# MrTornado24/IDE-3D

Measured on AMD Instinct MI355X. Metric: 512x512 RGB+seg frames/s @96 depth samples (whole job), higher is better.
Workload: dtype f32 (3x3 convs + MLPs: fp32 operands as 3 bf16 pieces, 6 products, f32 accumulate); 1 GPU; BASELINE config 2: random-init ide3d-ffhq-64-512, G.mapping + G.synthesis (64 render -> 512, 96 samples, RGB + 19-class seg) + uint8 frames, batch 4 seeds per GPU; global_batch=4, parallelism=dp1, conv_arithmetic=bf16x6, conv_arithmetic_is_library_default=True

## Files before the change

### ide-3d_amd/csrc/upfirdn2d.hip

```cpp
#include "common.h"
#include "knobs.h"
#include <type_traits>

namespace ide3d {

template <class T>
__device__ __forceinline__ typename Elem<T>::math_t
apply_epilogue(typename Elem<T>::math_t v, const ide3d_upfirdn2d_epilogue& ep, int n, int c, int oy, int ox, int out_w) {
    using M = typename Elem<T>::math_t;
    if (ep.add) v += Elem<T>::ld((const T*)ep.add + n * ep.add_stride[0] + c * ep.add_stride[1] + oy * ep.add_stride[2] + ox * ep.add_stride[3]);
    if (ep.noise) v += (M)(ep.noise[oy * out_w + ox] * ep.noise_strength);
    if (ep.fused_act) {
        if (ep.bias) v += Elem<T>::ld((const T*)ep.bias + c);
        if (ep.act == 3) v = (v > 0) ? v : v * (M)ep.alpha;
        v *= (M)ep.act_gain;
        if (ep.clamp >= 0.f) v = (v > (M)ep.clamp) ? (M)ep.clamp : ((v < -(M)ep.clamp) ? -(M)ep.clamp : v);
    }
    return v;
}

template <class T, int NO>
__device__ __forceinline__ void epilogue_row(typename Elem<T>::math_t (&row)[NO], const ide3d_upfirdn2d_epilogue& ep,
                                             const T* add_plane, typename Elem<T>::math_t bias, int oy, int ox0, int out_w, bool full) {
    using M = typename Elem<T>::math_t;
    if (ep.add) {
        const T* ap = add_plane + (int64_t)oy * ep.add_stride[2];
        if constexpr (sizeof(T) == 4 && NO == 4) {
            if (full && ep.add_stride[3] == 1 && ((reinterpret_cast<uintptr_t>(ap + ox0) & 15) == 0)) {
                const float4 a = *reinterpret_cast<const float4*>(ap + ox0);
                row[0] += a.x; row[1] += a.y; row[2] += a.z; row[3] += a.w;
                goto add_done;
            }
        }
#pragma unroll
        for (int j = 0; j < NO; ++j) {
            const int ox = ox0 + j;
            if (ox >= 0 && ox < out_w) row[j] += Elem<T>::ld(ap + (int64_t)ox * ep.add_stride[3]);
        }
    }
add_done:
    if (ep.noise) {
        const float* np_ = ep.noise + (int64_t)oy * out_w;
        if (NO == 4 && full && ((reinterpret_cast<uintptr_t>(np_ + ox0) & 15) == 0)) {
            const float4 a = *reinterpret_cast<const float4*>(np_ + ox0);
            row[0] += (M)(a.x * ep.noise_strength); row[1] += (M)(a.y * ep.noise_strength);
            row[2] += (M)(a.z * ep.noise_strength); row[3] += (M)(a.w * ep.noise_strength);
        } else {
#pragma unroll
            for (int j = 0; j < NO; ++j) {
                const int ox = ox0 + j;
                if (ox >= 0 && ox < out_w) row[j] += (M)(np_[ox] * ep.noise_strength);
            }
        }
    }
    if (ep.fused_act) {
#pragma unroll
        for (int j = 0; j < NO; ++j) {
            M v = row[j] + bias;
            if (ep.act == 3) v = (v > 0) ? v : v * (M)ep.alpha;
            v *= (M)ep.act_gain;
            if (ep.clamp >= 0.f) v = (v > (M)ep.clamp) ? (M)ep.clamp : ((v < -(M)ep.clamp) ? -(M)ep.clamp : v);
            row[j] = v;
        }
    }
}


template <class T>
__global__ void __launch_bounds__(256)
upfirdn2d_generic_kernel(ide3d_upfirdn2d_params p, ide3d_upfirdn2d_epilogue ep, int c_fastest) {
    using M = typename Elem<T>::math_t;
    const T* __restrict__ x = (const T*)p.x;
    T* __restrict__ y = (T*)p.y;
    const int64_t total = (int64_t)p.n * p.c * p.out_h * p.out_w;
    const int64_t stride = (int64_t)gridDim.x * blockDim.x;
    int am_n = -1; float am = 0.f;
    __shared__ unsigned s_am[64];
    const bool am_lds = ep.y_amax && p.n <= 64;
    if (ep.y_amax) { if (threadIdx.x < 64) s_am[threadIdx.x] = 0u; __syncthreads(); }
    for (int64_t idx = (int64_t)blockIdx.x * blockDim.x + threadIdx.x; idx < total; idx += stride) {
        int ox, oy, c, n;
        int64_t r = idx;
        if (c_fastest) {
            c = (int)(r % p.c); r /= p.c;
            ox = (int)(r % p.out_w); r /= p.out_w;
            oy = (int)(r % p.out_h); r /= p.out_h;
            n = (int)r;
        } else {
            ox = (int)(r % p.out_w); r /= p.out_w;
            oy = (int)(r % p.out_h); r /= p.out_h;
            c = (int)(r % p.c); r /= p.c;
            n = (int)r;
        }
        const int X0 = ox * p.down_x - p.pad_x0;
        const int Y0 = oy * p.down_y - p.pad_y0;
        int kx0, ky0, ix0, iy0;
        if (p.up_x == 1) { kx0 = 0; ix0 = X0; } else { ix0 = floordiv(X0 + p.up_x - 1, p.up_x); kx0 = ix0 * p.up_x - X0; }
        if (p.up_y == 1) { ky0 = 0; iy0 = Y0; } else { iy0 = floordiv(Y0 + p.up_y - 1, p.up_y); ky0 = iy0 * p.up_y - Y0; }
        int ty_begin = 0, tx_begin = 0;
        if (iy0 < 0) ty_begin = -iy0;
        if (ix0 < 0) tx_begin = -ix0;
        const int ty_end = min((p.f_h - ky0 + p.up_y - 1) / p.up_y, p.in_h - iy0);
        const int tx_end = min((p.f_w - kx0 + p.up_x - 1) / p.up_x, p.in_w - ix0);
        const T* xp = x + n * p.x_stride[0] + c * p.x_stride[1];
        M acc = 0;
        for (int ty = ty_begin; ty < ty_end; ++ty) {
            const int ky = ky0 + ty * p.up_y;
            const int fy = p.flip ? ky : p.f_h - 1 - ky;
            const T* xr = xp + (int64_t)(iy0 + ty) * p.x_stride[2];
            const float* fr = p.f + (int64_t)fy * p.f_stride[0];
            int kx = kx0 + tx_begin * p.up_x;
            for (int tx = tx_begin; tx < tx_end; ++tx, kx += p.up_x) {
                const int fx = p.flip ? kx : p.f_w - 1 - kx;
                acc += Elem<T>::ld(xr + (int64_t)(ix0 + tx) * p.x_stride[3]) * (M)fr[fx * p.f_stride[1]];
            }
        }
        const M out = apply_epilogue<T>(acc * (M)p.gain, ep, n, c, oy, ox, p.out_w);
        Elem<T>::st(y + n * p.y_stride[0] + c * p.y_stride[1] + oy * p.y_stride[2] + ox * p.y_stride[3], out);
        if (ep.y_amax) {
            if (n != am_n) { if (am_n >= 0) { if (am_lds) amax_lds_flush(s_am, am_n, am); else if (am > 0.f) amax_raise(ep.y_amax, am_n, am); } am_n = n; am = 0.f; }
            am = fmaxf(am, fabsf((float)out));
        }
    }
    if (ep.y_amax) {
        if (am_n >= 0) { if (am_lds) amax_lds_flush(s_am, am_n, am); else if (am > 0.f) amax_raise(ep.y_amax, am_n, am); }
        if (am_lds) amax_lds_commit(ep.y_amax, s_am, p.n);
    }
}

__host__ __device__ inline int cell_row_floats(int ntx, int U) { return ((ntx + 1 + 7) / 8) * 8 * U; }

template <class T, int U>
__global__ void __launch_bounds__(256)
upfirdn2d_cell_kernel(ide3d_upfirdn2d_params p, ide3d_upfirdn2d_epilogue ep, int cells_x, int cells_y, int qx_min, int qy_min, int ntx, int nty) {
    using M = typename Elem<T>::math_t;
    extern __shared__ __attribute__((aligned(16))) float s_fpad[];
    const int FPW = cell_row_floats(ntx, U), FPH = (nty + 1) * U;
    for (int e = threadIdx.x; e < FPW * FPH; e += 256) {
        const int ky = e / FPW - (U - 1), kx = e % FPW - (U - 1);
        float v = 0.f;
        if (ky >= 0 && ky < p.f_h && kx >= 0 && kx < p.f_w) {
            const int fy = p.flip ? ky : p.f_h - 1 - ky, fx = p.flip ? kx : p.f_w - 1 - kx;
            v = p.f[(int64_t)fy * p.f_stride[0] + (int64_t)fx * p.f_stride[1]];
        }
        s_fpad[e] = v;
    }
    __syncthreads();
    const T* __restrict__ x = (const T*)p.x;
    T* __restrict__ y = (T*)p.y;
    const int64_t total = (int64_t)p.n * p.c * cells_y * U * cells_x;
    const int64_t stride = (int64_t)gridDim.x * blockDim.x;
    for (int64_t idx = (int64_t)blockIdx.x * blockDim.x + threadIdx.x; idx < total; idx += stride) {
        int64_t r = idx;
        const int cxi = (int)(r % cells_x); r /= cells_x;
        const int jy = (int)(r % U); r /= U;
        const int cyi = (int)(r % cells_y); r /= cells_y;
        const int c = (int)(r % p.c), n = (int)(r / p.c);
        const int qx = qx_min + cxi, qy = qy_min + cyi;
        const int oy = qy * U + jy + p.pad_y0;
        if (oy < 0 || oy >= p.out_h) continue;
        M acc[U];
#pragma unroll
        for (int jx = 0; jx < U; ++jx) acc[jx] = 0;
        const T* xp = x + n * p.x_stride[0] + c * p.x_stride[1];
        for (int dy = 0; dy <= nty; ++dy) {
            const int iy = qy + dy;
            if (iy < 0 || iy >= p.in_h) continue;
            const T* xr = xp + (int64_t)iy * p.x_stride[2];
            const float* frow = s_fpad + (dy * U + U - 1 - jy) * FPW;
            const int s3 = (int)p.x_stride[3];
            for (int dx0 = 0; dx0 <= ntx; dx0 += 8) {
                M xv[8];
#pragma unroll
                for (int e = 0; e < 8; ++e) {
                    const int ix = qx + dx0 + e;
                    const bool ok = (unsigned)ix < (unsigned)p.in_w;
                    const M v = Elem<T>::ld(xr + (ok ? ix : 0) * s3);
                    xv[e] = ok ? v : (M)0;
                }
                const float* fb = frow + dx0 * U;
#pragma unroll
                for (int e = 0; e < 8; ++e) {
#pragma unroll
                    for (int jx = 0; jx < U; ++jx) acc[jx] += xv[e] * (M)fb[e * U + U - 1 - jx];
                }
            }
        }
#pragma unroll
        for (int jx = 0; jx < U; ++jx) {
            const int ox = qx * U + jx + p.pad_x0;
            if (ox < 0 || ox >= p.out_w) continue;
            const M out = apply_epilogue<T>(acc[jx] * (M)p.gain, ep, n, c, oy, ox, p.out_w);
            Elem<T>::st(y + n * p.y_stride[0] + c * p.y_stride[1] + oy * p.y_stride[2] + ox * p.y_stride[3], out);
        }
    }
}


template <int U, int D, int F>
struct Axis {
    static constexpr int NT = (F + U - 1) / U;
    static constexpr int first(int r) { return (U - r) % U; }
    static constexpr int ntaps(int r) { return first(r) < F ? (F - first(r) + U - 1) / U : 0; }
    static constexpr int off(int r) { return r == 0 ? 0 : 1; }
    static constexpr int window(int C) { return U > 1 ? C + NT : (C - 1) * D + F; }
    static constexpr int step = (U > 1) ? 1 : D;
};

template <int UX, int UY, int DX, int DY, int FW, int FH, int CX, int CY>
struct TileGeom {
    using AX = Axis<UX, DX, FW>;
    using AY = Axis<UY, DY, FH>;
    static constexpr int TX = 32, TY = 8;
    static constexpr int TCX = TX * CX, TCY = TY * CY;
    static constexpr int LW = ((AX::window(TCX) + 3) & ~3) + 4;
    static constexpr int LH = AY::window(TCY);
    static constexpr int NLD4 = (LH * (LW / 4) + 255) / 256;
};

__host__ __device__ constexpr bool tile_stage16_instance(int elem_bytes, int nld4) { return elem_bytes == 4 && nld4 <= 16; }
__host__ __device__ inline bool tile_stage16_plane(int64_t pitch, int in_w, int x_row_floats, uintptr_t plane_addr) {
    const int w4 = (in_w + 3) & ~3;
    return (pitch & 3) == 0 && pitch >= w4 && w4 <= (in_w > x_row_floats ? in_w : x_row_floats) && (plane_addr & 15) == 0;
}

template <class T, int UX, int UY, int DX, int DY, int FW, int FH, int CX, int CY>
__global__ void __launch_bounds__(256)
upfirdn2d_tile_kernel(ide3d_upfirdn2d_params p, ide3d_upfirdn2d_epilogue ep, int tiles_x, int tiles_y) {
    using M = typename Elem<T>::math_t;
    using G = TileGeom<UX, UY, DX, DY, FW, FH, CX, CY>;
    using AX = typename G::AX;
    using AY = typename G::AY;
    constexpr int TX = G::TX;
    constexpr int TCX = G::TCX, TCY = G::TCY;
    constexpr int LW = G::LW, LH = G::LH;
    constexpr int WX = AX::window(CX), WY = AY::window(CY);

    __shared__ __attribute__((aligned(16))) M s_in[LH * LW];

    M g[FH][FW];
#pragma unroll
    for (int ky = 0; ky < FH; ++ky)
#pragma unroll
        for (int kx = 0; kx < FW; ++kx) {
            const int fy = p.flip ? ky : FH - 1 - ky;
            const int fx = p.flip ? kx : FW - 1 - kx;
            g[ky][kx] = (M)p.f[fy * p.f_stride[0] + fx * p.f_stride[1]] * (M)p.gain;
        }

    const int nblocks = gridDim.x;
    int bid = xcd_remap(blockIdx.x, nblocks);
    const int tx_i = bid % tiles_x; bid /= tiles_x;
    const int ty_i = bid % tiles_y; bid /= tiles_y;
    const int plane = bid;
    const int n = plane / p.c, c = plane % p.c;

    const int qx_min = (UX > 1) ? floordiv(-p.pad_x0, UX) : 0;
    const int qy_min = (UY > 1) ? floordiv(-p.pad_y0, UY) : 0;
    const int qx0 = qx_min + tx_i * TCX;
    const int qy0 = qy_min + ty_i * TCY;
    const int in_x0 = (UX > 1) ? qx0 : qx0 * DX - p.pad_x0;
    const int in_y0 = (UY > 1) ? qy0 : qy0 * DY - p.pad_y0;

    const T* __restrict__ xp = (const T*)p.x + n * p.x_stride[0] + c * p.x_stride[1];
    int xoff = 0;
    bool staged = false;
    if constexpr (tile_stage16_instance((int)sizeof(T), G::NLD4)) {
        const int64_t pitch = p.x_stride[2];
        const int w4 = (p.in_w + 3) & ~3;
        if (tile_stage16_plane(pitch, p.in_w, p.x_row_floats, reinterpret_cast<uintptr_t>(xp))) {
            const int x_al = in_x0 & ~3;
            xoff = in_x0 - x_al;
            constexpr int NV = LW / 4, NLD4 = (LH * NV + 255) / 256;
            static_assert(LW % 4 == 0 && LW >= AX::window(TCX) + 4, "LDS rows hold the window shifted by up to 3 columns");
            float4 v4[NLD4];
            unsigned long long okb = 0;
#pragma unroll
            for (int k = 0; k < NLD4; ++k) {
                const int idx = (int)threadIdx.x + k * 256;
                const int ly = idx / NV, lv = idx - ly * NV;
                const int gy = in_y0 + ly, gx = x_al + 4 * lv;
                const int cy_ = min(max(gy, 0), p.in_h - 1), cxv = min(max(gx, 0), w4 - 4);
                v4[k] = *reinterpret_cast<const float4*>(reinterpret_cast<const float*>(xp) + (int64_t)cy_ * pitch + cxv);
                const bool rowok = (gy == cy_) && idx < LH * NV;
#pragma unroll
                for (int e = 0; e < 4; ++e) okb |= (rowok && gx + e >= 0 && gx + e < p.in_w) ? (1ull << (4 * k + e)) : 0ull;
            }
#pragma unroll
            for (int k = 0; k < NLD4; ++k) {
                const int idx = (int)threadIdx.x + k * 256;
                if (idx < LH * NV) {
                    float4 w = v4[k];
                    w.x = ((okb >> (4 * k + 0)) & 1ull) ? w.x : 0.f; w.y = ((okb >> (4 * k + 1)) & 1ull) ? w.y : 0.f;
                    w.z = ((okb >> (4 * k + 2)) & 1ull) ? w.z : 0.f; w.w = ((okb >> (4 * k + 3)) & 1ull) ? w.w : 0.f;
                    *reinterpret_cast<float4*>(reinterpret_cast<float*>(s_in) + 4 * idx) = w;
                }
            }
            staged = true;
        }
    }
    if (!staged) {
        constexpr int NLD = (LH * LW + 255) / 256;
        constexpr int DROW = 256 / LW, DCOL = 256 % LW;
        M v[NLD];
        int ly = (int)threadIdx.x / LW, lx = (int)threadIdx.x % LW;
        static_assert(NLD <= 64, "staging loads per thread must fit the validity mask");
        unsigned long long okbits = 0;
#pragma unroll
        for (int k = 0; k < NLD; ++k) {
            const int iy = in_y0 + ly, ix = in_x0 + lx;
            const int cy_ = min(max(iy, 0), p.in_h - 1), cx_ = min(max(ix, 0), p.in_w - 1);
            v[k] = Elem<T>::ld(xp + cy_ * p.x_stride[2] + cx_);
            okbits |= (lx < AX::window(TCX) && iy == cy_ && ix == cx_ && ly < LH) ? (1ull << k) : 0ull;
            lx += DCOL; ly += DROW;
            if (lx >= LW) { lx -= LW; ++ly; }
        }
#pragma unroll
        for (int k = 0; k < NLD; ++k) {
            const int i = (int)threadIdx.x + k * 256;
            if (i < LH * LW) s_in[i] = ((okbits >> k) & 1ull) ? v[k] : (M)0;
        }
    }
    __syncthreads();

    const int tx = threadIdx.x % TX, ty = threadIdx.x / TX;
    M win[WY][WX];
    const int lx0 = tx * CX * AX::step, ly0 = ty * CY * AY::step;
#pragma unroll
    for (int wy = 0; wy < WY; ++wy)
#pragma unroll
        for (int wx = 0; wx < WX; ++wx)
            win[wy][wx] = s_in[(ly0 + wy) * LW + lx0 + xoff + wx];

    float amax_t = 0.f;
    T* __restrict__ yp = (T*)p.y + n * p.y_stride[0] + c * p.y_stride[1];
    const T* add_plane = ep.add ? (const T*)ep.add + (int64_t)n * ep.add_stride[0] + (int64_t)c * ep.add_stride[1] : nullptr;
    const M bias = (ep.fused_act && ep.bias) ? (M)Elem<T>::ld((const T*)ep.bias + c) : (M)0;
#pragma unroll
    for (int cy = 0; cy < CY; ++cy)
#pragma unroll
        for (int ry = 0; ry < UY; ++ry) {
            const int qy = qy0 + ty * CY + cy;
            const int oy = (UY > 1) ? qy * UY + ry + p.pad_y0 : qy;
            if (oy < 0 || oy >= p.out_h) continue;
            M row[CX * UX];
#pragma unroll
            for (int cx = 0; cx < CX; ++cx)
#pragma unroll
                for (int rx = 0; rx < UX; ++rx) {
                    M acc = 0;
#pragma unroll
                    for (int ty_ = 0; ty_ < AY::ntaps(ry); ++ty_)
#pragma unroll
                        for (int tx_ = 0; tx_ < AX::ntaps(rx); ++tx_) {
                            const int wy = (UY > 1) ? cy + AY::off(ry) + ty_ : cy * DY + ty_;
                            const int wx = (UX > 1) ? cx + AX::off(rx) + tx_ : cx * DX + tx_;
                            acc += win[wy][wx] * g[AY::first(ry) + ty_ * UY][AX::first(rx) + tx_ * UX];
                        }
                    row[cx * UX + rx] = acc;
                }
            const int qx = qx0 + tx * CX;
            const int ox0 = (UX > 1) ? qx * UX + p.pad_x0 : qx;
            T* yr = yp + oy * p.y_stride[2];
            constexpr int NO = CX * UX;
            const bool full = ox0 >= 0 && ox0 + NO <= p.out_w;
            epilogue_row<T, NO>(row, ep, add_plane, bias, oy, ox0, p.out_w, full);
#pragma unroll
            for (int j = 0; j < NO; ++j)
                if (full || (ox0 + j >= 0 && ox0 + j < p.out_w)) amax_t = fmaxf(amax_t, fabsf((float)row[j]));
            if constexpr (sizeof(T) == 4 && NO == 4) {
                if (full && ((reinterpret_cast<uintptr_t>(yr + ox0) & 15) == 0)) {
                    float4 v4 = make_float4(row[0], row[1], row[2], row[3]);
                    *reinterpret_cast<float4*>(yr + ox0) = v4;
                    continue;
                }
            }
#pragma unroll
            for (int j = 0; j < NO; ++j) {
                const int ox = ox0 + j;
                if (ox >= 0 && ox < p.out_w) Elem<T>::st(yr + ox, row[j]);
            }
        }
    if (ep.y_amax) amax_raise_block(ep.y_amax, n, amax_t, reinterpret_cast<float*>(s_in));
}

__global__ void __launch_bounds__(256)
fir44_kernel(ide3d_upfirdn2d_params p, ide3d_upfirdn2d_epilogue ep, int tiles_x, int tiles_y) {
    constexpr int TCX = 128, TCY = 32, LW = 136, LH = TCY + 3, NV = LW / 4, NLD = (LH * NV + 255) / 256;
    __shared__ __attribute__((aligned(16))) float s_in[LH * LW];
    float g[4][4];
#pragma unroll
    for (int ky = 0; ky < 4; ++ky)
#pragma unroll
        for (int kx = 0; kx < 4; ++kx) {
            const int fy = p.flip ? ky : 3 - ky, fx = p.flip ? kx : 3 - kx;
            g[ky][kx] = p.f[fy * p.f_stride[0] + fx * p.f_stride[1]] * p.gain;
        }
    int bid = xcd_remap(blockIdx.x, gridDim.x);
    const int tx_i = bid % tiles_x; bid /= tiles_x;
    const int ty_i = bid % tiles_y; bid /= tiles_y;
    const int n = bid / p.c, c = bid % p.c;
    const int in_x0 = tx_i * TCX - p.pad_x0, in_y0 = ty_i * TCY - p.pad_y0;
    const int x_al = in_x0 & ~3, xoff = in_x0 - x_al;
    const float* __restrict__ xp = (const float*)p.x + n * p.x_stride[0] + c * p.x_stride[1];
    const unsigned pitch = (unsigned)p.x_stride[2];
    const int w4 = (p.in_w + 3) & ~3;
    {
        float4 v4[NLD];
        int gy[NLD], gx[NLD];
#pragma unroll
        for (int k = 0; k < NLD; ++k) {
            const int idx = (int)threadIdx.x + k * 256;
            const int ly = idx / NV, lv = idx - ly * NV;
            gy[k] = in_y0 + ly; gx[k] = x_al + 4 * lv;
            const unsigned cy_ = (unsigned)min(max(gy[k], 0), p.in_h - 1), cx_ = (unsigned)min(max(gx[k], 0), w4 - 4);
            v4[k] = *reinterpret_cast<const float4*>(xp + (cy_ * pitch + cx_));
        }
#pragma unroll
        for (int k = 0; k < NLD; ++k) {
            const int idx = (int)threadIdx.x + k * 256;
            if (idx < LH * NV) {
                const bool rowok = (unsigned)gy[k] < (unsigned)p.in_h;
                float4 w = v4[k];
                w.x = (rowok && (unsigned)(gx[k] + 0) < (unsigned)p.in_w) ? w.x : 0.f;
                w.y = (rowok && (unsigned)(gx[k] + 1) < (unsigned)p.in_w) ? w.y : 0.f;
                w.z = (rowok && (unsigned)(gx[k] + 2) < (unsigned)p.in_w) ? w.z : 0.f;
                w.w = (rowok && (unsigned)(gx[k] + 3) < (unsigned)p.in_w) ? w.w : 0.f;
                *reinterpret_cast<float4*>(s_in + 4 * idx) = w;
            }
        }
    }
    __syncthreads();
    const int tx = threadIdx.x & 31, ty = threadIdx.x >> 5;
    float win[7][7];
    {
        const float* wsrc = s_in + (ty * 4) * LW + tx * 4 + xoff;
#pragma unroll
        for (int wy = 0; wy < 7; ++wy)
#pragma unroll
            for (int wx = 0; wx < 7; ++wx) win[wy][wx] = wsrc[wy * LW + wx];
    }
    const bool has_noise = ep.noise != nullptr, act_on = ep.fused_act != 0;
    const float nstr = ep.noise_strength;
    const float bias = (act_on && ep.bias) ? ((const float*)ep.bias)[c] : 0.f;
    const bool lrelu = act_on && ep.act == 3, lrelu_max = lrelu && ep.alpha >= 0.f && ep.alpha <= 1.f;
    const float alpha = ep.alpha, again = act_on ? ep.act_gain : 1.f;
    const bool clamp_on = act_on && ep.clamp >= 0.f;
    const float cl = ep.clamp;
    float* __restrict__ yp = (float*)p.y + n * p.y_stride[0] + c * p.y_stride[1];
    const unsigned ypitch = (unsigned)p.y_stride[2];
    const int ox0 = tx_i * TCX + tx * 4, oy0 = ty_i * TCY + ty * 4;
    const bool full = ox0 + 4 <= p.out_w;
    float amax_t = 0.f;
    if (full) {
#pragma unroll
        for (int cy = 0; cy < 4; ++cy) {
            const int oy = oy0 + cy;
            if (oy >= p.out_h) break;
            float row[4];
#pragma unroll
            for (int cx = 0; cx < 4; ++cx) {
                float acc = 0.f;
#pragma unroll
                for (int ky = 0; ky < 4; ++ky)
#pragma unroll
                    for (int kx = 0; kx < 4; ++kx) acc += win[cy + ky][cx + kx] * g[ky][kx];
                row[cx] = acc;
            }
            if (has_noise) {
                const float4 a = *reinterpret_cast<const float4*>(ep.noise + ((unsigned)oy * (unsigned)p.out_w + (unsigned)ox0));
                row[0] += a.x * nstr; row[1] += a.y * nstr; row[2] += a.z * nstr; row[3] += a.w * nstr;
            }
            if (act_on) {
#pragma unroll
                for (int j = 0; j < 4; ++j) {
                    float v = row[j] + bias;
                    if (lrelu_max) v = fmaxf(v, v * alpha);
                    else if (lrelu) v = (v > 0.f) ? v : v * alpha;
                    v *= again;
                    if (clamp_on) v = (v > cl) ? cl : ((v < -cl) ? -cl : v);
                    row[j] = v;
                }
            }
#pragma unroll
            for (int j = 0; j < 4; ++j) amax_t = fmaxf(amax_t, fabsf(row[j]));
            *reinterpret_cast<float4*>(yp + ((unsigned)oy * ypitch + (unsigned)ox0)) = make_float4(row[0], row[1], row[2], row[3]);
        }
    }
    if (ep.y_amax) amax_raise_block(ep.y_amax, n, amax_t, s_in);
}

__global__ void __launch_bounds__(256)
fir_up2_kernel(ide3d_upfirdn2d_params p, ide3d_upfirdn2d_epilogue ep, int tiles_x, int tiles_y) {
    using AX = Axis<2, 1, 4>;
    constexpr int TCX = 64, TCY = 16, LW = 72, LH = TCY + 2, NV = LW / 4, NLD = (LH * NV + 255) / 256;
    static_assert(AX::window(TCX) + 3 <= LW && AX::NT == 2 && AX::window(2) == 4, "window of the 4-tap polyphase filter");
    __shared__ __attribute__((aligned(16))) float s_in[LH * LW];
    float g[4][4];
#pragma unroll
    for (int ky = 0; ky < 4; ++ky)
#pragma unroll
        for (int kx = 0; kx < 4; ++kx) {
            const int fy = p.flip ? ky : 3 - ky, fx = p.flip ? kx : 3 - kx;
            g[ky][kx] = p.f[fy * p.f_stride[0] + fx * p.f_stride[1]] * p.gain;
        }
    int bid = xcd_remap(blockIdx.x, gridDim.x);
    const int tx_i = bid % tiles_x; bid /= tiles_x;
    const int ty_i = bid % tiles_y; bid /= tiles_y;
    const int n = bid / p.c, c = bid % p.c;
    const int qx0 = floordiv(-p.pad_x0, 2) + tx_i * TCX, qy0 = floordiv(-p.pad_y0, 2) + ty_i * TCY;
    const int x_al = qx0 & ~3, xoff = qx0 - x_al;
    const float* __restrict__ xp = (const float*)p.x + n * p.x_stride[0] + c * p.x_stride[1];
    const unsigned pitch = (unsigned)p.x_stride[2];
    const int w4 = (p.in_w + 3) & ~3;
    {
        float4 v4[NLD];
        int gy[NLD], gx[NLD];
#pragma unroll
        for (int k = 0; k < NLD; ++k) {
            const int idx = (int)threadIdx.x + k * 256;
            const int ly = idx / NV, lv = idx - ly * NV;
            gy[k] = qy0 + ly; gx[k] = x_al + 4 * lv;
            const unsigned cy_ = (unsigned)min(max(gy[k], 0), p.in_h - 1), cx_ = (unsigned)min(max(gx[k], 0), w4 - 4);
            v4[k] = *reinterpret_cast<const float4*>(xp + (cy_ * pitch + cx_));
        }
#pragma unroll
        for (int k = 0; k < NLD; ++k) {
            const int idx = (int)threadIdx.x + k * 256;
            if (idx < LH * NV) {
                const bool rowok = (unsigned)gy[k] < (unsigned)p.in_h;
                float4 w = v4[k];
                w.x = (rowok && (unsigned)(gx[k] + 0) < (unsigned)p.in_w) ? w.x : 0.f;
                w.y = (rowok && (unsigned)(gx[k] + 1) < (unsigned)p.in_w) ? w.y : 0.f;
                w.z = (rowok && (unsigned)(gx[k] + 2) < (unsigned)p.in_w) ? w.z : 0.f;
                w.w = (rowok && (unsigned)(gx[k] + 3) < (unsigned)p.in_w) ? w.w : 0.f;
                *reinterpret_cast<float4*>(s_in + 4 * idx) = w;
            }
        }
    }
    __syncthreads();
    const int tx = threadIdx.x & 31, ty = threadIdx.x >> 5;
    float win[4][4];
    {
        const float* wsrc = s_in + (ty * 2) * LW + tx * 2 + xoff;
#pragma unroll
        for (int wy = 0; wy < 4; ++wy)
#pragma unroll
            for (int wx = 0; wx < 4; ++wx) win[wy][wx] = wsrc[wy * LW + wx];
    }
    const bool has_add = ep.add != nullptr, has_noise = ep.noise != nullptr, act_on = ep.fused_act != 0;
    const float nstr = ep.noise_strength;
    const float bias = (act_on && ep.bias) ? ((const float*)ep.bias)[c] : 0.f;
    const bool lrelu = act_on && ep.act == 3, lrelu_max = lrelu && ep.alpha >= 0.f && ep.alpha <= 1.f;
    const float alpha = ep.alpha, again = act_on ? ep.act_gain : 1.f;
    const bool clamp_on = act_on && ep.clamp >= 0.f;
    const float cl = ep.clamp;
    float* __restrict__ yp = (float*)p.y + n * p.y_stride[0] + c * p.y_stride[1];
    const float* __restrict__ ap = has_add ? (const float*)ep.add + n * ep.add_stride[0] + c * ep.add_stride[1] : nullptr;
    const unsigned ypitch = (unsigned)p.y_stride[2], apitch = (unsigned)ep.add_stride[2];
    const int ox0 = (qx0 + tx * 2) * 2 + p.pad_x0;
    const bool full = ox0 >= 0 && ox0 + 4 <= p.out_w;
    float amax_t = 0.f;
    if (full) {
#pragma unroll
        for (int cy = 0; cy < 2; ++cy)
#pragma unroll
            for (int ry = 0; ry < 2; ++ry) {
                const int oy = (qy0 + ty * 2 + cy) * 2 + ry + p.pad_y0;
                if (oy < 0 || oy >= p.out_h) continue;
                float row[4];
#pragma unroll
                for (int cx = 0; cx < 2; ++cx)
#pragma unroll
                    for (int rx = 0; rx < 2; ++rx) {
                        float acc = 0.f;
#pragma unroll
                        for (int ty_ = 0; ty_ < 2; ++ty_)
#pragma unroll
                            for (int tx_ = 0; tx_ < 2; ++tx_)
                                acc += win[cy + AX::off(ry) + ty_][cx + AX::off(rx) + tx_] * g[AX::first(ry) + ty_ * 2][AX::first(rx) + tx_ * 2];
                        row[cx * 2 + rx] = acc;
                    }
                if (has_add) {
                    const float4 a = *reinterpret_cast<const float4*>(ap + ((unsigned)oy * apitch + (unsigned)ox0));
                    row[0] += a.x; row[1] += a.y; row[2] += a.z; row[3] += a.w;
                }
                if (has_noise) {
                    const float4 a = *reinterpret_cast<const float4*>(ep.noise + ((unsigned)oy * (unsigned)p.out_w + (unsigned)ox0));
                    row[0] += a.x * nstr; row[1] += a.y * nstr; row[2] += a.z * nstr; row[3] += a.w * nstr;
                }
                if (act_on) {
#pragma unroll
                    for (int j = 0; j < 4; ++j) {
                        float v = row[j] + bias;
                        if (lrelu_max) v = fmaxf(v, v * alpha);
                        else if (lrelu) v = (v > 0.f) ? v : v * alpha;
                        v *= again;
                        if (clamp_on) v = (v > cl) ? cl : ((v < -cl) ? -cl : v);
                        row[j] = v;
                    }
                }
#pragma unroll
                for (int j = 0; j < 4; ++j) amax_t = fmaxf(amax_t, fabsf(row[j]));
                *reinterpret_cast<float4*>(yp + ((unsigned)oy * ypitch + (unsigned)ox0)) = make_float4(row[0], row[1], row[2], row[3]);
            }
    }
    if (ep.y_amax) amax_raise_block(ep.y_amax, n, amax_t, s_in);
}


static bool fir44_applies(const ide3d_upfirdn2d_params& p, const ide3d_upfirdn2d_epilogue& ep) {
    const bool off = knob_live("IDE3D_FIR_NO_LEAN");
    if (off || p.dtype != IDE3D_F32 || p.f_w != 4 || p.f_h != 4 || p.up_x != 1 || p.up_y != 1 || p.down_x != 1 || p.down_y != 1) return false;
    if (p.x_stride[3] != 1 || p.y_stride[3] != 1 || ep.add || p.out_w <= 64 || (p.out_w & 3)) return false;
    const int64_t pitch = p.x_stride[2], w4 = (p.in_w + 3) & ~3;
    if ((pitch & 3) || pitch < w4 || w4 > (p.in_w > p.x_row_floats ? p.in_w : p.x_row_floats)) return false;
    if ((reinterpret_cast<uintptr_t>(p.x) & 15) || (p.x_stride[0] & 3) || (p.x_stride[1] & 3)) return false;
    if ((reinterpret_cast<uintptr_t>(p.y) & 15) || (p.y_stride[0] & 3) || (p.y_stride[1] & 3) || (p.y_stride[2] & 3)) return false;
    if (ep.noise && (reinterpret_cast<uintptr_t>(ep.noise) & 15)) return false;
    if (pitch * p.in_h >= (1ll << 29) || p.y_stride[2] * (int64_t)p.out_h >= (1ll << 29) || (int64_t)p.out_w * p.out_h >= (1ll << 29)) return false;
    if (p.x_stride[2] <= 0 || p.y_stride[2] <= 0) return false;
    return true;
}

static bool fir_up2_applies(const ide3d_upfirdn2d_params& p, const ide3d_upfirdn2d_epilogue& ep) {
    const bool off = knob_live("IDE3D_FIR_NO_LEAN");
    if (off || p.dtype != IDE3D_F32 || p.f_w != 4 || p.f_h != 4 || p.up_x != 2 || p.up_y != 2 || p.down_x != 1 || p.down_y != 1) return false;
    if (p.x_stride[3] != 1 || p.y_stride[3] != 1 || (p.out_w & 3) || (p.in_w & 3)) return false;
    if (p.pad_x0 & 1) return false;
    const int64_t pitch = p.x_stride[2];
    if ((pitch & 3) || pitch < p.in_w || pitch <= 0 || p.y_stride[2] <= 0) return false;
    if ((reinterpret_cast<uintptr_t>(p.x) & 15) || (p.x_stride[0] & 3) || (p.x_stride[1] & 3)) return false;
    if ((reinterpret_cast<uintptr_t>(p.y) & 15) || (p.y_stride[0] & 3) || (p.y_stride[1] & 3) || (p.y_stride[2] & 3)) return false;
    if (ep.add && (ep.add_stride[3] != 1 || (reinterpret_cast<uintptr_t>(ep.add) & 15) || (ep.add_stride[0] & 3) || (ep.add_stride[1] & 3) || (ep.add_stride[2] & 3) ||
                   ep.add_stride[2] <= 0 || ep.add_stride[2] * (int64_t)p.out_h >= (1ll << 29))) return false;
    if (ep.noise && (reinterpret_cast<uintptr_t>(ep.noise) & 15)) return false;
    if (pitch * p.in_h >= (1ll << 29) || p.y_stride[2] * (int64_t)p.out_h >= (1ll << 29) || (int64_t)p.out_w * p.out_h >= (1ll << 29)) return false;
    return true;
}

static bool cell_applies(const ide3d_upfirdn2d_params& p, const ide3d_upfirdn2d_epilogue& ep) {
    if (knob_live("IDE3D_FIR_NO_CELL")) return false;
    if (p.up_x != p.up_y || (p.up_x != 2 && p.up_x != 4) || p.down_x != 1 || p.down_y != 1 || ep.y_amax) return false;
    if ((int64_t)p.f_w * p.f_h < 36) return false;
    const int U = p.up_x;
    return (int64_t)cell_row_floats(cdiv(p.f_w, U), U) * (cdiv(p.f_h, U) + 1) * U * 4 <= 48 * 1024 && p.x_stride[3] * (int64_t)p.in_w < (1ll << 31);
}

static inline int cells_of(int out, int pad0, int U) {
    if (U == 1) return out;
    return floordiv(out - 1 - pad0, U) - floordiv(-pad0, U) + 1;
}

static int tile_staging(const ide3d_upfirdn2d_params& p) {
    int staged = 0, planes = 0;
    for (int n = 0; n < (p.n < 4 ? p.n : 4); ++n)
        for (int c = 0; c < (p.c < 4 ? p.c : 4); ++c, ++planes)
            staged += tile_stage16_plane(p.x_stride[2], p.in_w, p.x_row_floats,
                                         reinterpret_cast<uintptr_t>(p.x) + (uintptr_t)((n * p.x_stride[0] + c * p.x_stride[1]) * 4)) ? 1 : 0;
    return staged == planes ? 1 : staged == 0 ? 0 : 2;
}

template <int UX, int UY, int DX, int DY, int FW, int FH, int CX, int CY>
static int plan_tile(const ide3d_upfirdn2d_params& p, ide3d_upfirdn2d_plan_info* o) {
    using G = TileGeom<UX, UY, DX, DY, FW, FH, CX, CY>;
    o->form = IDE3D_UPFIRDN_TILE;
    o->ux = UX; o->uy = UY; o->dx = DX; o->dy = DY; o->fw = FW; o->fh = FH; o->cx = CX; o->cy = CY;
    o->tiles_x = cdiv(cells_of(p.out_w, p.pad_x0, UX), G::TCX);
    o->tiles_y = cdiv(cells_of(p.out_h, p.pad_y0, UY), G::TCY);
    o->grid = (int64_t)o->tiles_x * o->tiles_y * p.n * p.c;
    o->staging = (p.dtype == IDE3D_F32 && tile_stage16_instance(4, G::NLD4)) ? tile_staging(p) : 0;
    if (o->grid > 0x7fffffff) { set_error("upfirdn2d: grid too large"); return IDE3D_EINVAL; }
    return IDE3D_OK;
}

static int upfirdn2d_plan(const ide3d_upfirdn2d_params& p, const ide3d_upfirdn2d_epilogue& ep, ide3d_upfirdn2d_plan_info* o) {
    *o = ide3d_upfirdn2d_plan_info{};
    o->staging = -1;
    const bool w_contig = (p.x_stride[3] == 1 && p.y_stride[3] == 1);
    const bool f32 = p.dtype == IDE3D_F32;
    if (p.dtype != IDE3D_F64) {
        if (w_contig && p.f_w == 4 && p.f_h == 4) {
            if (p.up_x == 1 && p.up_y == 1 && p.down_x == 1 && p.down_y == 1) {
                if (p.out_w <= 64) return plan_tile<1, 1, 1, 1, 4, 4, 2, 4>(p, o);
                if (f32 && fir44_applies(p, ep)) {
                    o->form = IDE3D_UPFIRDN_FIR44;
                    o->ux = 1; o->uy = 1; o->dx = 1; o->dy = 1; o->fw = 4; o->fh = 4; o->cx = 4; o->cy = 4;
                    o->staging = 1;
                    o->tiles_x = cdiv(p.out_w, 128); o->tiles_y = cdiv(p.out_h, 32);
                    o->grid = (int64_t)o->tiles_x * o->tiles_y * p.n * p.c;
                    if (o->grid > 0x7fffffff) { set_error("upfirdn2d: grid too large"); return IDE3D_EINVAL; }
                    return IDE3D_OK;
                }
                return plan_tile<1, 1, 1, 1, 4, 4, 4, 4>(p, o);
            }
            if (p.up_x == 2 && p.up_y == 2 && p.down_x == 1 && p.down_y == 1) {
                if (f32 && fir_up2_applies(p, ep)) {
                    o->form = IDE3D_UPFIRDN_FIR_UP2;
                    o->ux = 2; o->uy = 2; o->dx = 1; o->dy = 1; o->fw = 4; o->fh = 4; o->cx = 2; o->cy = 2;
                    o->staging = 1;
                    o->tiles_x = cdiv(cells_of(p.out_w, p.pad_x0, 2), 64); o->tiles_y = cdiv(cells_of(p.out_h, p.pad_y0, 2), 16);
                    o->grid = (int64_t)o->tiles_x * o->tiles_y * p.n * p.c;
                    if (o->grid > 0x7fffffff) { set_error("upfirdn2d: grid too large"); return IDE3D_EINVAL; }
                    return IDE3D_OK;
                }
                return plan_tile<2, 2, 1, 1, 4, 4, 2, 2>(p, o);
            }
            if (p.up_x == 1 && p.up_y == 1 && p.down_x == 2 && p.down_y == 2) return plan_tile<1, 1, 2, 2, 4, 4, 4, 2>(p, o);
        }
        if (f32) {
            if (w_contig && p.f_w == 12 && p.f_h == 1 && p.up_y == 1 && p.down_y == 1) {
                if (p.up_x == 2 && p.down_x == 1) return plan_tile<2, 1, 1, 1, 12, 1, 2, 4>(p, o);
                if (p.up_x == 1 && p.down_x == 2) return plan_tile<1, 1, 2, 1, 12, 1, 4, 4>(p, o);
                if (p.up_x == 1 && p.down_x == 1) return plan_tile<1, 1, 1, 1, 12, 1, 4, 4>(p, o);
            }
            if (w_contig && p.f_w == 1 && p.f_h == 12 && p.up_x == 1 && p.down_x == 1) {
                if (p.up_y == 2 && p.down_y == 1) return plan_tile<1, 2, 1, 1, 1, 12, 4, 2>(p, o);
                if (p.up_y == 1 && p.down_y == 2) return plan_tile<1, 1, 1, 2, 1, 12, 4, 2>(p, o);
                if (p.up_y == 1 && p.down_y == 1) return plan_tile<1, 1, 1, 1, 1, 12, 4, 4>(p, o);
            }
        }
        if (cell_applies(p, ep)) {
            const int U = p.up_x;
            o->form = IDE3D_UPFIRDN_CELL;
            o->cell_u = U;
            o->tiles_x = cells_of(p.out_w, p.pad_x0, U); o->tiles_y = cells_of(p.out_h, p.pad_y0, U);
            o->lds_bytes = (int64_t)cell_row_floats(cdiv(p.f_w, U), U) * (cdiv(p.f_h, U) + 1) * U * (int64_t)sizeof(float);
            o->grid = stream_grid((int64_t)p.n * p.c * o->tiles_y * U * o->tiles_x, 256);
            return IDE3D_OK;
        }
    }
    o->form = IDE3D_UPFIRDN_GENERIC;
    o->c_fastest = (p.y_stride[1] == 1 && p.c > 1) ? 1 : 0;
    o->grid = stream_grid((int64_t)p.n * p.c * p.out_h * p.out_w, 256);
    return IDE3D_OK;
}

template <class T, int UX, int UY, int DX, int DY, int FW, int FH, int CX, int CY>
static int launch_tile(const ide3d_upfirdn2d_params& p, const ide3d_upfirdn2d_epilogue& ep, const ide3d_upfirdn2d_plan_info& pl, hipStream_t st) {
    hipLaunchKernelGGL((upfirdn2d_tile_kernel<T, UX, UY, DX, DY, FW, FH, CX, CY>), dim3((unsigned)pl.grid),
                       dim3(256), 0, st, p, ep, pl.tiles_x, pl.tiles_y);
    IDE3D_CHECK_LAUNCH("upfirdn2d_tile");
    return IDE3D_OK;
}

template <class T, int U>
static int launch_cell(const ide3d_upfirdn2d_params& p, const ide3d_upfirdn2d_epilogue& ep, const ide3d_upfirdn2d_plan_info& pl, hipStream_t st) {
    hipLaunchKernelGGL((upfirdn2d_cell_kernel<T, U>), dim3((unsigned)pl.grid), dim3(256), (size_t)pl.lds_bytes, st, p, ep, pl.tiles_x, pl.tiles_y,
                       floordiv(-p.pad_x0, U), floordiv(-p.pad_y0, U), cdiv(p.f_w, U), cdiv(p.f_h, U));
    IDE3D_CHECK_LAUNCH("upfirdn2d_cell");
    return IDE3D_OK;
}

template <class T>
static int launch_planned(const ide3d_upfirdn2d_params& p, const ide3d_upfirdn2d_epilogue& ep, const ide3d_upfirdn2d_plan_info& pl, hipStream_t st) {
#define IDE3D_TILE_CASE(UX, UY, DX, DY, FW, FH, CX, CY)                                                                              \
    if (pl.ux == UX && pl.uy == UY && pl.dx == DX && pl.dy == DY && pl.fw == FW && pl.fh == FH && pl.cx == CX && pl.cy == CY)         \
        return launch_tile<T, UX, UY, DX, DY, FW, FH, CX, CY>(p, ep, pl, st)
    switch (pl.form) {
    case IDE3D_UPFIRDN_FIR44:
        if constexpr (std::is_same<T, float>::value) {
            hipLaunchKernelGGL(fir44_kernel, dim3((unsigned)pl.grid), dim3(256), 0, st, p, ep, pl.tiles_x, pl.tiles_y);
            IDE3D_CHECK_LAUNCH("upfirdn2d (fir44)");
            return IDE3D_OK;
        }
        break;
    case IDE3D_UPFIRDN_FIR_UP2:
        if constexpr (std::is_same<T, float>::value) {
            hipLaunchKernelGGL(fir_up2_kernel, dim3((unsigned)pl.grid), dim3(256), 0, st, p, ep, pl.tiles_x, pl.tiles_y);
            IDE3D_CHECK_LAUNCH("upfirdn2d (fir_up2)");
            return IDE3D_OK;
        }
        break;
    case IDE3D_UPFIRDN_TILE:
        if constexpr (!std::is_same<T, double>::value) {
            IDE3D_TILE_CASE(1, 1, 1, 1, 4, 4, 2, 4);
            IDE3D_TILE_CASE(1, 1, 1, 1, 4, 4, 4, 4);
            IDE3D_TILE_CASE(2, 2, 1, 1, 4, 4, 2, 2);
            IDE3D_TILE_CASE(1, 1, 2, 2, 4, 4, 4, 2);
        }
        if constexpr (std::is_same<T, float>::value) {
            IDE3D_TILE_CASE(2, 1, 1, 1, 12, 1, 2, 4);
            IDE3D_TILE_CASE(1, 1, 2, 1, 12, 1, 4, 4);
            IDE3D_TILE_CASE(1, 1, 1, 1, 12, 1, 4, 4);
            IDE3D_TILE_CASE(1, 2, 1, 1, 1, 12, 4, 2);
            IDE3D_TILE_CASE(1, 1, 1, 2, 1, 12, 4, 2);
            IDE3D_TILE_CASE(1, 1, 1, 1, 1, 12, 4, 4);
        }
        break;
    case IDE3D_UPFIRDN_CELL:
        if constexpr (!std::is_same<T, double>::value) return pl.cell_u == 2 ? launch_cell<T, 2>(p, ep, pl, st) : launch_cell<T, 4>(p, ep, pl, st);
        break;
    case IDE3D_UPFIRDN_GENERIC:
        hipLaunchKernelGGL((upfirdn2d_generic_kernel<T>), dim3((unsigned)pl.grid), dim3(256), 0, st, p, ep, pl.c_fastest);
        IDE3D_CHECK_LAUNCH("upfirdn2d_generic");
        return IDE3D_OK;
    }
#undef IDE3D_TILE_CASE
    set_error("upfirdn2d: no kernel for the planned form %d", pl.form);
    return IDE3D_ENOKERNEL;
}

}

static int upfirdn2d_checked_plan(const ide3d_upfirdn2d_params* pp, const ide3d_upfirdn2d_epilogue* epp, ide3d_upfirdn2d_epilogue* ep_out,
                                  ide3d_upfirdn2d_plan_info* plan) {
    using namespace ide3d;
    IDE3D_CHECK_ARG(pp != nullptr, "upfirdn2d: null params");
    const ide3d_upfirdn2d_params& p = *pp;
    ide3d_upfirdn2d_epilogue ep{};
    if (epp) ep = *epp;
    IDE3D_CHECK_ARG(p.x && p.f && p.y, "upfirdn2d: null tensor pointer");
    IDE3D_CHECK_ARG(p.n > 0 && p.c > 0 && p.in_h > 0 && p.in_w > 0, "upfirdn2d: x is empty");
    IDE3D_CHECK_ARG(p.f_h >= 1 && p.f_w >= 1, "upfirdn2d: f is empty");
    IDE3D_CHECK_ARG(p.up_x >= 1 && p.up_y >= 1, "upfirdn2d: upsampling factor must be at least 1");
    IDE3D_CHECK_ARG(p.down_x >= 1 && p.down_y >= 1, "upfirdn2d: downsampling factor must be at least 1");
    IDE3D_CHECK_ARG(p.out_h >= 1 && p.out_w >= 1, "upfirdn2d: output must be at least 1x1");
    IDE3D_CHECK_ARG(!ep.fused_act || ep.act == 1 || ep.act == 3, "upfirdn2d_ex: fused activation must be linear (1) or lrelu (3)");
    if (p.dtype != IDE3D_F32 && p.dtype != IDE3D_F16 && p.dtype != IDE3D_BF16 && p.dtype != IDE3D_F64) {
        set_error("upfirdn2d: unsupported dtype code %d", p.dtype);
        return IDE3D_EINVAL;
    }
    *ep_out = ep;
    return upfirdn2d_plan(p, ep, plan);
}

static int upfirdn2d_entry(const ide3d_upfirdn2d_params* pp, const ide3d_upfirdn2d_epilogue* epp, void* stream) {
    using namespace ide3d;
    ide3d_upfirdn2d_epilogue ep;
    ide3d_upfirdn2d_plan_info plan;
    const int rc = upfirdn2d_checked_plan(pp, epp, &ep, &plan);
    if (rc != IDE3D_OK) return rc;
    const ide3d_upfirdn2d_params& p = *pp;
    hipStream_t st = (hipStream_t)stream;
    switch (p.dtype) {
    case IDE3D_F32:  return launch_planned<float>(p, ep, plan, st);
    case IDE3D_F16:  return launch_planned<__half>(p, ep, plan, st);
    case IDE3D_BF16: return launch_planned<__hip_bfloat16>(p, ep, plan, st);
    default:         return launch_planned<double>(p, ep, plan, st);
    }
}

extern "C" int ide3d_upfirdn2d_plan(const ide3d_upfirdn2d_params* pp, const ide3d_upfirdn2d_epilogue* epp, ide3d_upfirdn2d_plan_info* out) {
    using namespace ide3d;
    IDE3D_CHECK_ARG(out, "upfirdn2d_plan: null pointer");
    ide3d_upfirdn2d_epilogue ep;
    return upfirdn2d_checked_plan(pp, epp, &ep, out);
}

extern "C" int ide3d_upfirdn2d(const ide3d_upfirdn2d_params* pp, void* stream) {
    return upfirdn2d_entry(pp, nullptr, stream);
}

extern "C" int ide3d_upfirdn2d_ex(const ide3d_upfirdn2d_params* pp, const ide3d_upfirdn2d_epilogue* ep, void* stream) {
    return upfirdn2d_entry(pp, ep, stream);
}
```

Before: 936.8 frames/s.

## Restructure fir44 kernel: pipelined LDS row reads, compile-time x offset, magic division

The 4x4 FIR kernel is templated on the x misalignment so window indexing becomes compile-time. Each row is loaded with inline-asm ds_read_b128 and explicit lgkmcnt waits, issued one row ahead, and the FMAs are accumulated row by row instead of first loading a full 7x7 scalar window. Block-index decomposition now uses precomputed magic-number division, filter taps are loaded once per lane and broadcast with readlane, and noise loads are hoisted ahead of the LDS fill. The intent is to cut LDS instruction count, integer divide cost and register pressure. Hand-written waitcnt asm adds fragility if the compiler reorders other LDS ops.

```diff
diff --git a/ide-3d_amd/csrc/upfirdn2d.hip b/ide-3d_amd/csrc/upfirdn2d.hip
--- a/ide-3d_amd/csrc/upfirdn2d.hip
+++ b/ide-3d_amd/csrc/upfirdn2d.hip
@@ -384,27 +384,86 @@
     if (ep.y_amax) amax_raise_block(ep.y_amax, n, amax_t, reinterpret_cast<float*>(s_in));
 }
 
+typedef float fir_f4 __attribute__((ext_vector_type(4)));
+template <int OFF, int NQ>
+__device__ __forceinline__ void fir_row_read(fir_f4 (&q)[NQ], unsigned addr) {
+    asm volatile("ds_read_b128 %0, %1 offset:%2" : "=v"(q[0]) : "v"(addr), "n"(OFF));
+    asm volatile("ds_read_b128 %0, %1 offset:%2" : "=v"(q[1]) : "v"(addr), "n"(OFF + 16));
+    if constexpr (NQ == 3) asm volatile("ds_read_b128 %0, %1 offset:%2" : "=v"(q[2]) : "v"(addr), "n"(OFF + 32));
+}
+template <int N, int NQ>
+__device__ __forceinline__ void fir_row_wait(fir_f4 (&q)[NQ], fir_f4 (&acc)[4]) {
+    if constexpr (NQ == 3) asm volatile("s_waitcnt lgkmcnt(%7)" : "+v"(q[0]), "+v"(q[1]), "+v"(q[2]), "+v"(acc[0]), "+v"(acc[1]), "+v"(acc[2]), "+v"(acc[3]) : "n"(N));
+    else asm volatile("s_waitcnt lgkmcnt(%6)" : "+v"(q[0]), "+v"(q[1]), "+v"(acc[0]), "+v"(acc[1]), "+v"(acc[2]), "+v"(acc[3]) : "n"(N));
+}
+template <int PITCH, int NQ>
+__device__ __forceinline__ void fir_row_issue(fir_f4 (&q)[NQ], unsigned addr, int r) {
+    switch (r) {
+    case 0: fir_row_read<0 * PITCH>(q, addr); break;
+    case 1: fir_row_read<1 * PITCH>(q, addr); break;
+    case 2: fir_row_read<2 * PITCH>(q, addr); break;
+    case 3: fir_row_read<3 * PITCH>(q, addr); break;
+    case 4: fir_row_read<4 * PITCH>(q, addr); break;
+    case 5: fir_row_read<5 * PITCH>(q, addr); break;
+    default: fir_row_read<6 * PITCH>(q, addr); break;
+    }
+}
+template <int NQ>
+__device__ __forceinline__ void fir_row_await(fir_f4 (&q)[NQ], fir_f4 (&acc)[4], int rows_behind) {
+    switch (rows_behind) {
+    case 2: fir_row_wait<2 * NQ>(q, acc); break;
+    case 1: fir_row_wait<NQ>(q, acc); break;
+    default: fir_row_wait<0>(q, acc); break;
+    }
+}
+
+struct FirDiv { unsigned m; int sh; };
+static FirDiv fir_div_of(int d) {
+    int l = 0;
+    while ((1ll << l) < d) ++l;
+    return FirDiv{(unsigned)((1ull << (31 + l)) / (unsigned long long)d + 1ull), 31 + l};
+}
+__device__ __forceinline__ int fir_div(int n, FirDiv d) { return (int)(((unsigned long long)(unsigned)n * d.m) >> d.sh); }
+
+template <int XOFF>
 __global__ void __launch_bounds__(256)
-fir44_kernel(ide3d_upfirdn2d_params p, ide3d_upfirdn2d_epilogue ep, int tiles_x, int tiles_y) {
+fir44_kernel(ide3d_upfirdn2d_params p, ide3d_upfirdn2d_epilogue ep, int tiles_x, int tiles_y, FirDiv div_tx, FirDiv div_ty, FirDiv div_c) {
     constexpr int TCX = 128, TCY = 32, LW = 136, LH = TCY + 3, NV = LW / 4, NLD = (LH * NV + 255) / 256;
+    constexpr int NQ = (XOFF + 7 + 3) / 4;
+    static_assert(31 * 4 + 4 * NQ <= LW, "the last lane's quads end inside the LDS row");
     __shared__ __attribute__((aligned(16))) float s_in[LH * LW];
-    float g[4][4];
-#pragma unroll
-    for (int ky = 0; ky < 4; ++ky)
-#pragma unroll
-        for (int kx = 0; kx < 4; ++kx) {
-            const int fy = p.flip ? ky : 3 - ky, fx = p.flip ? kx : 3 - kx;
-            g[ky][kx] = p.f[fy * p.f_stride[0] + fx * p.f_stride[1]] * p.gain;
-        }
-    int bid = xcd_remap(blockIdx.x, gridDim.x);
-    const int tx_i = bid % tiles_x; bid /= tiles_x;
-    const int ty_i = bid % tiles_y; bid /= tiles_y;
-    const int n = bid / p.c, c = bid % p.c;
+    float gl;
+    {
+        const int kl = (int)threadIdx.x & 15, ky_l = kl >> 2, kx_l = kl & 3;
+        const int fy = p.flip ? ky_l : 3 - ky_l, fx = p.flip ? kx_l : 3 - kx_l;
+        gl = p.f[fy * p.f_stride[0] + fx * p.f_stride[1]] * p.gain;
+    }
+    const int bid = xcd_remap(blockIdx.x, gridDim.x);
+    const int b1 = fir_div(bid, div_tx), tx_i = bid - b1 * tiles_x;
+    const int b2 = fir_div(b1, div_ty), ty_i = b1 - b2 * tiles_y;
+    const int n = fir_div(b2, div_c), c = b2 - n * p.c;
     const int in_x0 = tx_i * TCX - p.pad_x0, in_y0 = ty_i * TCY - p.pad_y0;
-    const int x_al = in_x0 & ~3, xoff = in_x0 - x_al;
+    const int x_al = in_x0 - XOFF;
     const float* __restrict__ xp = (const float*)p.x + n * p.x_stride[0] + c * p.x_stride[1];
     const unsigned pitch = (unsigned)p.x_stride[2];
     const int w4 = (p.in_w + 3) & ~3;
+    const bool has_noise = ep.noise != nullptr, act_on = ep.fused_act != 0;
+    const float nstr = ep.noise_strength;
+    const float bias = (act_on && ep.bias) ? ((const float*)ep.bias)[c] : 0.f;
+    const bool lrelu = act_on && ep.act == 3, lrelu_max = lrelu && ep.alpha >= 0.f && ep.alpha <= 1.f;
+    const float alpha = ep.alpha, again = ep.act_gain;
+    const bool clamp_on = act_on && ep.clamp >= 0.f;
+    const float cl = ep.clamp;
+    const int tx = threadIdx.x & 31, ty = threadIdx.x >> 5;
+    const int ox0 = tx_i * TCX + tx * 4, oy0 = ty_i * TCY + ty * 4;
+    const bool full = ox0 + 4 <= p.out_w;
+    const int nrows = min(max(p.out_h - oy0, 0), 4);
+    float4 nz[4];
+    if (has_noise) {
+#pragma unroll
+        for (int cy = 0; cy < 4; ++cy)
+            nz[cy] = *reinterpret_cast<const float4*>(ep.noise + ((unsigned)min(oy0 + cy, p.out_h - 1) * (unsigned)p.out_w + (unsigned)(full ? ox0 : 0)));
+    }
     {
         float4 v4[NLD];
         int gy[NLD], gx[NLD];
@@ -431,61 +490,72 @@
         }
     }
     __syncthreads();
-    const int tx = threadIdx.x & 31, ty = threadIdx.x >> 5;
-    float win[7][7];
-    {
-        const float* wsrc = s_in + (ty * 4) * LW + tx * 4 + xoff;
-#pragma unroll
-        for (int wy = 0; wy < 7; ++wy)
-#pragma unroll
-            for (int wx = 0; wx < 7; ++wx) win[wy][wx] = wsrc[wy * LW + wx];
-    }
-    const bool has_noise = ep.noise != nullptr, act_on = ep.fused_act != 0;
-    const float nstr = ep.noise_strength;
-    const float bias = (act_on && ep.bias) ? ((const float*)ep.bias)[c] : 0.f;
-    const bool lrelu = act_on && ep.act == 3, lrelu_max = lrelu && ep.alpha >= 0.f && ep.alpha <= 1.f;
-    const float alpha = ep.alpha, again = act_on ? ep.act_gain : 1.f;
-    const bool clamp_on = act_on && ep.clamp >= 0.f;
-    const float cl = ep.clamp;
+    float g[4][4];
+#pragma unroll
+    for (int ky = 0; ky < 4; ++ky)
+#pragma unroll
+        for (int kx = 0; kx < 4; ++kx) g[ky][kx] = __int_as_float(__builtin_amdgcn_readlane(__float_as_int(gl), ky * 4 + kx));
     float* __restrict__ yp = (float*)p.y + n * p.y_stride[0] + c * p.y_stride[1];
     const unsigned ypitch = (unsigned)p.y_stride[2];
-    const int ox0 = tx_i * TCX + tx * 4, oy0 = ty_i * TCY + ty * 4;
-    const bool full = ox0 + 4 <= p.out_w;
     float amax_t = 0.f;
-    if (full) {
-#pragma unroll
-        for (int cy = 0; cy < 4; ++cy) {
-            const int oy = oy0 + cy;
-            if (oy >= p.out_h) break;
-            float row[4];
-#pragma unroll
-            for (int cx = 0; cx < 4; ++cx) {
-                float acc = 0.f;
-#pragma unroll
-                for (int ky = 0; ky < 4; ++ky)
-#pragma unroll
-                    for (int kx = 0; kx < 4; ++kx) acc += win[cy + ky][cx + kx] * g[ky][kx];
-                row[cx] = acc;
-            }
-            if (has_noise) {
-                const float4 a = *reinterpret_cast<const float4*>(ep.noise + ((unsigned)oy * (unsigned)p.out_w + (unsigned)ox0));
-                row[0] += a.x * nstr; row[1] += a.y * nstr; row[2] += a.z * nstr; row[3] += a.w * nstr;
-            }
-            if (act_on) {
-#pragma unroll
-                for (int j = 0; j < 4; ++j) {
-                    float v = row[j] + bias;
-                    if (lrelu_max) v = fmaxf(v, v * alpha);
-                    else if (lrelu) v = (v > 0.f) ? v : v * alpha;
-                    v *= again;
-                    if (clamp_on) v = (v > cl) ? cl : ((v < -cl) ? -cl : v);
-                    row[j] = v;
-                }
-            }
-#pragma unroll
-            for (int j = 0; j < 4; ++j) amax_t = fmaxf(amax_t, fabsf(row[j]));
-            *reinterpret_cast<float4*>(yp + ((unsigned)oy * ypitch + (unsigned)ox0)) = make_float4(row[0], row[1], row[2], row[3]);
-        }
+    if (full && nrows > 0) {
+        const unsigned wsrc = (unsigned)(uintptr_t)(__attribute__((address_space(3))) float*)s_in + (unsigned)(((ty * 4) * LW + tx * 4) * 4);
+        fir_f4 acc[4];
+#pragma unroll
+        for (int cy = 0; cy < 4; ++cy) acc[cy] = fir_f4{0.f, 0.f, 0.f, 0.f};
+        fir_f4 w[7][NQ];
+        constexpr int AHEAD = 1;
+        static_assert(AHEAD >= 1 && AHEAD <= 2, "fir_row_await knows 0, 1 and 2 rows in flight");
+#pragma unroll
+        for (int r = 0; r < AHEAD; ++r) fir_row_issue<LW * 4>(w[r], wsrc, r);
+#pragma unroll
+        for (int r = 0; r < 7; ++r) {
+            if (r + AHEAD < 7) fir_row_issue<LW * 4>(w[r + AHEAD], wsrc, r + AHEAD);
+            fir_row_await(w[r], acc, (6 - r < AHEAD ? 6 - r : AHEAD));
+            float wr[4 * NQ];
+#pragma unroll
+            for (int q = 0; q < NQ; ++q) { wr[4 * q] = w[r][q].x; wr[4 * q + 1] = w[r][q].y; wr[4 * q + 2] = w[r][q].z; wr[4 * q + 3] = w[r][q].w; }
+#pragma unroll
+            for (int cy = 0; cy < 4; ++cy) {
+                const int ky = r - cy;
+                if (ky < 0 || ky > 3) continue;
+#pragma unroll
+                for (int cx = 0; cx < 4; ++cx)
+#pragma unroll
+                    for (int kx = 0; kx < 4; ++kx) acc[cy][cx] += wr[XOFF + cx + kx] * g[ky][kx];
+            }
+        }
+        if (has_noise) {
+#pragma unroll
+            for (int cy = 0; cy < 4; ++cy) {
+                acc[cy][0] += nz[cy].x * nstr; acc[cy][1] += nz[cy].y * nstr; acc[cy][2] += nz[cy].z * nstr; acc[cy][3] += nz[cy].w * nstr;
+            }
+        }
+        if (act_on) {
+            if (lrelu_max) {
+#pragma unroll
+                for (int i = 0; i < 16; ++i) { float v = acc[i >> 2][i & 3] + bias; v = fmaxf(v, v * alpha); acc[i >> 2][i & 3] = v * again; }
+            } else if (lrelu) {
+#pragma unroll
+                for (int i = 0; i < 16; ++i) { float v = acc[i >> 2][i & 3] + bias; v = (v > 0.f) ? v : v * alpha; acc[i >> 2][i & 3] = v * again; }
+            } else {
+#pragma unroll
+                for (int i = 0; i < 16; ++i) { const float v = acc[i >> 2][i & 3] + bias; acc[i >> 2][i & 3] = v * again; }
+            }
+            if (clamp_on) {
+#pragma unroll
+                for (int i = 0; i < 16; ++i) { const float v = acc[i >> 2][i & 3]; acc[i >> 2][i & 3] = (v > cl) ? cl : ((v < -cl) ? -cl : v); }
+            }
+        }
+#pragma unroll
+        for (int cy = 0; cy < 4; ++cy)
+            if (cy < nrows) {
+                if (ep.y_amax) {
+#pragma unroll
+                    for (int j = 0; j < 4; ++j) amax_t = fmaxf(amax_t, fabsf(acc[cy][j]));
+                }
+                *reinterpret_cast<float4*>(yp + ((unsigned)(oy0 + cy) * ypitch + (unsigned)ox0)) = make_float4(acc[cy][0], acc[cy][1], acc[cy][2], acc[cy][3]);
+            }
     }
     if (ep.y_amax) amax_raise_block(ep.y_amax, n, amax_t, s_in);
 }
@@ -760,7 +830,13 @@
     switch (pl.form) {
     case IDE3D_UPFIRDN_FIR44:
         if constexpr (std::is_same<T, float>::value) {
-            hipLaunchKernelGGL(fir44_kernel, dim3((unsigned)pl.grid), dim3(256), 0, st, p, ep, pl.tiles_x, pl.tiles_y);
+            const FirDiv dtx = fir_div_of(pl.tiles_x), dty = fir_div_of(pl.tiles_y), dc = fir_div_of(p.c);
+            switch ((-p.pad_x0) & 3) {
+            case 0:  hipLaunchKernelGGL(fir44_kernel<0>, dim3((unsigned)pl.grid), dim3(256), 0, st, p, ep, pl.tiles_x, pl.tiles_y, dtx, dty, dc); break;
+            case 1:  hipLaunchKernelGGL(fir44_kernel<1>, dim3((unsigned)pl.grid), dim3(256), 0, st, p, ep, pl.tiles_x, pl.tiles_y, dtx, dty, dc); break;
+            case 2:  hipLaunchKernelGGL(fir44_kernel<2>, dim3((unsigned)pl.grid), dim3(256), 0, st, p, ep, pl.tiles_x, pl.tiles_y, dtx, dty, dc); break;
+            default: hipLaunchKernelGGL(fir44_kernel<3>, dim3((unsigned)pl.grid), dim3(256), 0, st, p, ep, pl.tiles_x, pl.tiles_y, dtx, dty, dc); break;
+            }
             IDE3D_CHECK_LAUNCH("upfirdn2d (fir44)");
             return IDE3D_OK;
         }
```

After: 941.3 frames/s, median of 6. No clear change (+0.5%).
